# HKUDS/SSLRec

Measured on AMD Instinct MI355X. Metric: propagation_edges_per_sec, higher is better.
Workload: dtype f32

## Files before the change

include/sslrec_hip.h:

```cpp
#ifndef SSLREC_HIP_H
#define SSLREC_HIP_H

#include <stddef.h>
#include <stdint.h>

#ifdef __cplusplus
extern "C" {
#endif

#define SSLREC_ABI_VERSION 7
#define SSLREC_E_BADARG 1001

int sslrec_abi_version(void);

int sslrec_row_bits3(const int64_t *idx0, int64_t off0, const int64_t *idx1, int64_t off1, const int64_t *idx2, int64_t off2,
                     int32_t n, int32_t n_rows, uint32_t *bits, void *stream);

typedef struct sslrec_csr {
    int32_t n_rows, n_cols, nnz;
    int32_t d;
    int32_t n_elem;
    const int32_t *col;
    const float   *val;
    int32_t n_waves;
// ... 118 lines not shown
                             int32_t *w_len_out, void *stream);

typedef struct sslrec_plan sslrec_plan_t;
#define SSLREC_PLAN_AUTO 0
#define SSLREC_PLAN_SWEPT 1
#define SSLREC_PLAN_STREAMED 2
#define SSLREC_PLAN_BUNDLED 3
#define SSLREC_PLAN_NO_XCD_SPLIT 1
typedef struct sslrec_plan_info {
    int32_t n_rows, n_cols; int64_t nnz;
    int32_t kind, d, xcd_split;
    int32_t n_elem, n_blocks, n_slots, n_streams, n_rseg, n_long;
    int64_t xcd_col_pairs;
} sslrec_plan_info_t;
int sslrec_plan_build_coo(const int64_t *rows, const int64_t *cols, const float *vals, int64_t nnz, int32_t n_rows,
                          int32_t n_cols, sslrec_plan_t **out);
int sslrec_plan_build_csr(const int64_t *rowptr, const int32_t *col, const float *val, int32_t n_rows, int32_t n_cols,
                          sslrec_plan_t **out);
int sslrec_plan_set_option(sslrec_plan_t *p, const char *name, int64_t value);
int sslrec_plan_layout(sslrec_plan_t *p, int32_t d, int32_t kind, int32_t flags);
int sslrec_plan_info(const sslrec_plan_t *p, int32_t d, int32_t kind, sslrec_plan_info_t *info);
int sslrec_plan_host_array(const sslrec_plan_t *p, int32_t d, int32_t kind, const char *name, const void **ptr, int64_t *count,
                           int32_t *elem_bytes);
int sslrec_plan_upload(sslrec_plan_t *p, int32_t d, int32_t kind, void *stream);
const sslrec_swept_t *sslrec_plan_swept(const sslrec_plan_t *p, int32_t d);
const sslrec_csr_t *sslrec_plan_csr(const sslrec_plan_t *p, int32_t d);
const sslrec_bundled_t *sslrec_plan_bundled(const sslrec_plan_t *p, int32_t d);
const int32_t *sslrec_plan_edge_map(const sslrec_plan_t *p, int32_t d, int32_t kind);
int sslrec_plan_spmm_f32(const sslrec_plan_t *p, int32_t d, const float *X, float *Y, const sslrec_epilogue_t *epi,
                         void *stream);
void sslrec_plan_free(sslrec_plan_t *p);

int sslrec_debug_swept_trace(int enable, unsigned long long *host_out, int n_waves);

int sslrec_debug_stamp_next_launch(unsigned long long *record);
int sslrec_debug_wall_clock_khz(void);

size_t sslrec_bpr_ws_bytes(int32_t B);
size_t sslrec_bpr_bwd_ws_bytes(int32_t B, int32_t d);
int sslrec_bpr_fwd_f32(const float *Ta, const int64_t *ia, const float *Tp, const int64_t *ip,
                       const float *Tn, const int64_t *in, int32_t B, int32_t d, int32_t variant,
                       float divisor, float *ws, float *loss_out, void *stream);
int sslrec_bpr_fwd_total_f32(const float *Ta, const int64_t *ia, const float *Tp, const int64_t *ip,
                             const float *Tn, const int64_t *in, int32_t B, int32_t d, int32_t variant,
                             float divisor, const float *add_in, float *ws, float *loss_out2, void *stream);
int sslrec_bpr_bwd_f32(const float *Ta, const int64_t *ia, const float *Tp, const int64_t *ip,
                       const float *Tn, const int64_t *in, int32_t B, int32_t d, int32_t variant, float divisor,
                       const float *gscale_dev, float *dTa, float *dTp, float *dTn, void *ws, void *stream);
int sslrec_bpr_bwd_table_init(void *ws, int32_t B, int32_t d, void *stream);
int sslrec_bpr_bwd_kept_f32(const float *Ta, const int64_t *ia, const float *Tp, const int64_t *ip,
                            const float *Tn, const int64_t *in, int32_t B, int32_t d, int32_t variant, float divisor,
                            const float *gscale_dev, float *dTa, float *dTp, float *dTn, void *ws, float *zero_table,
                            size_t zero_elems, void *stream);

#define SSLREC_INFONCE_PREC_DEFAULT 0
#define SSLREC_INFONCE_PREC_X6 1
#define SSLREC_INFONCE_PREC_FP32 2
#define SSLREC_INFONCE_PREC_X36 3
#define SSLREC_INFONCE_PREC_X3 4
#define SSLREC_INFONCE_PREC_X63 5
#define SSLREC_INFONCE_PREC_X6A 6
#define SSLREC_INFONCE_PREC_H3 7
#define SSLREC_INFONCE_FWD_W (1 << 16)
size_t sslrec_infonce_ws_bytes(int32_t B, int32_t M, int32_t d);
int sslrec_infonce_fwd_f32(const float *T1, const int64_t *i1, const float *T2, const int64_t *i2,
                           int32_t B, const float *ALL, int32_t M, int32_t d, float temp,
                           int32_t variant, float *ws, float *loss_out, void *stream);
int sslrec_infonce_bwd_f32(const float *T1, const int64_t *i1, const float *T2, const int64_t *i2,
                           int32_t B, const float *ALL, int32_t M, int32_t d, float temp,
                           int32_t variant, float *ws, const float *gscale_dev,
                           float *dE1, float *dE2, float *dALL, void *stream);

int sslrec_infonce_bwd_scatter_f32(const float *T1, const int64_t *i1, const float *T2, const int64_t *i2,
                                   int32_t B, const float *ALL, int32_t M, int32_t d, float temp,
                                   int32_t variant, float *ws, const float *gscale_dev, float *dE,
                                   float *dT1, float *dT2, float *dALL, void *scatter_ws, void *stream);

int sslrec_infonce_shard_rowsum_f32(const float *T1, const int64_t *i1, const float *T2, const int64_t *i2,
                                    int32_t B, const float *ALL, int32_t M, int32_t d, float temp,
                                    int32_t variant, float *ws, float *z_part, void *stream);
int sslrec_infonce_shard_loss_f32(int32_t B, int32_t M, int32_t d, int32_t variant, float *ws,
                                  const float *z_total, float *loss_out, void *stream);
int sslrec_infonce_shard_bwd_f32(int32_t B, int32_t M, int32_t d, float temp, int32_t variant, float *ws,
                                 const float *gscale_dev, float *w_part, float *dALL, void *stream);
int sslrec_infonce_shard_finish_bwd_f32(int32_t B, int32_t M, int32_t d, float temp, int32_t variant,
                                        float *ws, const float *gscale_dev, const float *w_total,
                                        float *dE1, float *dE2, void *stream);

size_t sslrec_sumsq_ws_bytes(void);
int sslrec_sumsq_fwd_f32(const float *x, size_t n, float weight, float *ws, float *out, void *stream);
int sslrec_sumsq_bwd_f32(const float *x, size_t n, float weight, const float *gscale_dev, float *dx, void *stream);

int sslrec_weighted_sum4_f32(const float *t0, float w0, const float *t1, float w1, const float *t2, float w2, const float *t3, float w3,
                             float *out6, void *stream);
int sslrec_scalar_scale2_f32(const float *x, float a, float b, float *out2, void *stream);
int sslrec_add_tables_f32(const float *a, const float *b, const float *c, float *out, size_t n, void *stream);

int sslrec_adam_tick(float *state, double lr, double beta1, double beta2, void *stream);
int sslrec_adam_apply_f32(float *p, const float *g, float *m, float *v, size_t n, const float *state,
                          double beta1, double beta2, double eps, double weight_decay, void *stream);

size_t sslrec_rankq_ws_bytes(int32_t q, int32_t d);
int sslrec_rankq_reduce_f32(const float *M, int64_t stride_q, int64_t stride_n, const float *X, int32_t N, int32_t d,
                            int32_t q, float *ws, float *out, void *stream);
int sslrec_rankq_expand_f32(const float *M, int64_t stride_q, int64_t stride_n, const float *S, int32_t N, int32_t d,
                            int32_t q, float *Y, void *stream);
// ... 27 lines not shown
```

sslrec_amd/_lib.py:

```python
import ctypes as C
import os
import subprocess

_HERE = os.path.dirname(os.path.abspath(__file__))
CSRC = os.path.join(_HERE, 'csrc')
SO_PATH = os.environ.get('SSLREC_HIP_LIBRARY') or os.path.join(CSRC, 'libsslrec_hip.so')

E_BADARG = 1001
EXPECTED_ABI = 7


class CsrStruct(C.Structure):
    _fields_ = [
        ('n_rows', C.c_int32), ('n_cols', C.c_int32), ('nnz', C.c_int32), ('d', C.c_int32), ('n_elem', C.c_int32),
        ('col', C.c_void_p), ('val', C.c_void_p),
        ('n_waves', C.c_int32),
        ('w_start', C.c_void_p), ('w_len', C.c_void_p), ('r_ptr', C.c_void_p),
        ('n_rseg', C.c_int32),
        ('r_len', C.c_void_p), ('r_dst', C.c_void_p),
        ('n_long', C.c_int32),
        ('long_row', C.c_void_p), ('long_ptr', C.c_void_p),
        ('n_slots', C.c_int32),
    ]

# ... 55 lines not shown
    'sslrec_debug_stamp_next_launch': (C.c_int, [C.c_void_p]),
    'sslrec_debug_wall_clock_khz': (C.c_int, []),
    'sslrec_philox_row_sumsq': (C.c_int, [_P, C.c_uint32, _I, _I, _P, _P]),
    'sslrec_row_sumsq_f32': (C.c_int, [_P, _I, _I, _P, _P]),
    'sslrec_debug_gather_rows': (C.c_int, [_P, C.c_uint32, _I, _I, _I, _P, _P, _P]),
    'sslrec_debug_swept_trace': (C.c_int, [C.c_int, _P, C.c_int]),
    'sslrec_spmm_csr_f32': (C.c_int, [C.POINTER(CsrStruct), _P, _P, _P, _P, _P, _I, _P, C.POINTER(EpilogueStruct), _P, _P]),
    'sslrec_spmm_bundled_f32': (C.c_int, [C.POINTER(BundledStruct), _P, _P, _I, _P, C.POINTER(EpilogueStruct), _P, _P]),
    'sslrec_spmm_swept_f32': (C.c_int, [C.POINTER(SweptStruct), _P, _P, _P, _P, _I, _P, C.POINTER(EpilogueStruct), _P]),
    'sslrec_swept_deferred_sum_ok': (C.c_int, [C.POINTER(SweptStruct)]),
    'sslrec_spmm_swept_views_f32': (C.c_int, [C.POINTER(SweptStruct), _P, _I, C.POINTER(EpilogueViewsStruct), _P]),
    'sslrec_swept_compact': (C.c_int, [C.POINTER(SweptStruct), _P, _P, _F, _P, _P, _P, _P]),
    'sslrec_edge_drop_compact': (C.c_int, [C.POINTER(CsrStruct), _P, _P, _F, _P, _P, _P, _P, _P]),
    'sslrec_full_predict_f32': (C.c_int, [_P, _P, _I, _P, _I, _I, _P, _I, _P, _P]),
    'sslrec_eval_topk_ws_bytes': (C.c_size_t, [_I, _I, _I]),
    'sslrec_eval_topk_f32': (C.c_int, [_P, _P, _I, _P, _I, _I, _P, _P, _I, _P, _P, _P, _P]),
    'sslrec_sample_negs': (C.c_int, [_P, C.c_int64, _P, _P, _I, _P, C.c_uint32, _P, _P]),
    'sslrec_sample_negs_mt19937': (C.c_int, [_P, _P, _P, C.c_int64, _P, _P, _I, _I, _P, _P]),
    'sslrec_philox_advance': (C.c_int, [_P, _P]),
    'sslrec_philox_fill_f32': (C.c_int, [_P, C.c_uint32, _P, C.c_size_t, _P]),
    'sslrec_mt19937_uniform_f32': (C.c_int, [_P, _P, C.c_int64, _P]),
    'sslrec_mt19937_keep_mask': (C.c_int, [_P, C.c_float, _P, C.c_int64, _P]),
    'sslrec_mt19937_jump_poly': (C.c_int, [_P, _P, _P, _P]),
    'sslrec_mt19937_par_ws_bytes': (C.c_size_t, [C.c_int32, C.c_int32]),
    'sslrec_mt19937_uniform_par_f32': (C.c_int, [_P, _P, C.c_int32, C.c_int32, C.c_int64, _P, _P, C.c_int64, _P]),
    'sslrec_mt19937_keep_mask_par': (C.c_int, [_P, _P, C.c_int32, C.c_int32, C.c_int64, _P, C.c_float, _P, C.c_int64, _P]),
    'sslrec_swept_compact_philox': (C.c_int, [C.POINTER(SweptStruct), _P, _F, _P, C.c_uint32, _F, _P, _P, _P, _P]),
    'sslrec_edge_drop_compact_philox': (C.c_int, [C.POINTER(CsrStruct), _P, _F, _P, C.c_uint32, _F, _P, _P, _P, _P, _P]),
    'sslrec_bundled_drop_values': (C.c_int, [C.POINTER(BundledStruct), _P, _P, _F, _P, C.c_uint32, _F, _P, _P]),
    'sslrec_bundled_compact': (C.c_int, [C.POINTER(BundledStruct), _P, _P, _F, _P, _P, _P, _P, _P]),
    'sslrec_bundled_compact_philox': (C.c_int, [C.POINTER(BundledStruct), _P, _F, _P, C.c_uint32, _F, _P, _P, _P, _P, _P]),
    'sslrec_spmm_bundled_view_f32': (C.c_int, [C.POINTER(BundledStruct), _P, _P, _P, _P, _P, _I, _P, C.POINTER(EpilogueStruct), _P, _P]),
    'sslrec_plan_build_coo': (C.c_int, [_P, _P, _P, C.c_int64, _I, _I, C.POINTER(C.c_void_p)]),
    'sslrec_plan_build_csr': (C.c_int, [_P, _P, _P, _I, _I, C.POINTER(C.c_void_p)]),
    'sslrec_plan_set_option': (C.c_int, [_P, C.c_char_p, C.c_int64]),
    'sslrec_plan_layout': (C.c_int, [_P, _I, _I, _I]),
    'sslrec_plan_info': (C.c_int, [_P, _I, _I, C.POINTER(PlanInfoStruct)]),
    'sslrec_plan_host_array': (C.c_int, [_P, _I, _I, C.c_char_p, C.POINTER(C.c_void_p), C.POINTER(C.c_int64), C.POINTER(C.c_int32)]),
    'sslrec_plan_upload': (C.c_int, [_P, _I, _I, _P]),
    'sslrec_plan_swept': (C.c_void_p, [_P, _I]),
    'sslrec_plan_csr': (C.c_void_p, [_P, _I]),
    'sslrec_plan_bundled': (C.c_void_p, [_P, _I]),
    'sslrec_plan_edge_map': (C.c_void_p, [_P, _I, _I]),
    'sslrec_plan_spmm_f32': (C.c_int, [_P, _I, _P, _P, C.POINTER(EpilogueStruct), _P]),
    'sslrec_plan_free': (None, [_P]),
    'sslrec_bpr_ws_bytes': (C.c_size_t, [_I]),
    'sslrec_bpr_fwd_f32': (C.c_int, [_P, _P, _P, _P, _P, _P, _I, _I, _I, _F, _P, _P, _P]),
    'sslrec_bpr_fwd_total_f32': (C.c_int, [_P, _P, _P, _P, _P, _P, _I, _I, _I, _F, _P, _P, _P, _P]),
    'sslrec_bpr_bwd_ws_bytes': (C.c_size_t, [_I, _I]),
    'sslrec_scatter_ws_bytes': (C.c_size_t, [_I]),
    'sslrec_bpr_bwd_f32': (C.c_int, [_P, _P, _P, _P, _P, _P, _I, _I, _I, _F, _P, _P, _P, _P, _P, _P]),
    'sslrec_bpr_bwd_table_init': (C.c_int, [_P, _I, _I, _P]),
    'sslrec_bpr_bwd_kept_f32': (C.c_int, [_P, _P, _P, _P, _P, _P, _I, _I, _I, _F, _P, _P, _P, _P, _P, _P, C.c_size_t, _P]),
    'sslrec_infonce_ws_bytes': (C.c_size_t, [_I, _I, _I]),
    'sslrec_infonce_fwd_f32': (C.c_int, [_P, _P, _P, _P, _I, _P, _I, _I, _F, _I, _P, _P, _P]),
    'sslrec_infonce_bwd_f32': (C.c_int, [_P, _P, _P, _P, _I, _P, _I, _I, _F, _I, _P, _P, _P, _P, _P, _P]),
    'sslrec_infonce_bwd_scatter_f32': (C.c_int, [_P, _P, _P, _P, _I, _P, _I, _I, _F, _I, _P, _P, _P, _P, _P, _P, _P, _P]),
    'sslrec_infonce_shard_rowsum_f32': (C.c_int, [_P, _P, _P, _P, _I, _P, _I, _I, _F, _I, _P, _P, _P]),
    'sslrec_infonce_shard_loss_f32': (C.c_int, [_I, _I, _I, _I, _P, _P, _P, _P]),
    'sslrec_infonce_shard_bwd_f32': (C.c_int, [_I, _I, _I, _F, _I, _P, _P, _P, _P, _P]),
    'sslrec_infonce_shard_finish_bwd_f32': (C.c_int, [_I, _I, _I, _F, _I, _P, _P, _P, _P, _P, _P]),
    'sslrec_adam_tick': (C.c_int, [_P, C.c_double, C.c_double, C.c_double, _P]),
    'sslrec_adam_apply_f32': (C.c_int, [_P, _P, _P, _P, C.c_size_t, _P, C.c_double, C.c_double, C.c_double, C.c_double, _P]),
    'sslrec_rankq_ws_bytes': (C.c_size_t, [_I, _I]),
    'sslrec_rankq_reduce_f32': (C.c_int, [_P, C.c_int64, C.c_int64, _P, _I, _I, _I, _P, _P, _P]),
    'sslrec_rankq_expand_f32': (C.c_int, [_P, C.c_int64, C.c_int64, _P, _I, _I, _I, _P, _P]),
    'sslrec_scatter_add_rows_f32': (C.c_int, [_P, _P, _I, _I, _P, _P, _P]),
    'sslrec_sumsq_ws_bytes': (C.c_size_t, []),
    'sslrec_sumsq_fwd_f32': (C.c_int, [_P, C.c_size_t, _F, _P, _P, _P]),
    'sslrec_sumsq_bwd_f32': (C.c_int, [_P, C.c_size_t, _F, _P, _P, _P]),
    'sslrec_weighted_sum4_f32': (C.c_int, [_P, _F, _P, _F, _P, _F, _P, _F, _P, _P]),
    'sslrec_scalar_scale2_f32': (C.c_int, [_P, _F, _F, _P, _P]),
    'sslrec_add_tables_f32': (C.c_int, [_P, _P, _P, _P, C.c_size_t, _P]),
}

_lib = None


def build(force=False):
    if force and os.path.exists(SO_PATH):
        os.remove(SO_PATH)
    subprocess.run(['make', '-C', CSRC], check=True)
    return SO_PATH


def load():
    global _lib
    if _lib is not None:
        return _lib
    if not os.path.exists(SO_PATH):
        raise RuntimeError(
            'libsslrec_hip.so is not built (%s). Run `python __graft_entry__.py` or `make -C sslrec_amd/csrc`. '
            'sslrec_amd has no CPU / PyTorch fallback for its kernels by design.' % SO_PATH)
    lib = C.CDLL(SO_PATH)
    for name, (res, args) in SIGNATURES.items():
        fn = getattr(lib, name)
        fn.restype = res
        fn.argtypes = args
    got = lib.sslrec_abi_version()
    if got != EXPECTED_ABI:
        raise RuntimeError('%s implements ABI version %d, these bindings expect %d: rebuild the library '
                           '(`make -C sslrec_amd/csrc` or `python __graft_entry__.py`)' % (SO_PATH, got, EXPECTED_ABI))
    _lib = lib
    return lib


# ... 5 lines not shown
```

sslrec_amd/csrc/losses.hip:

```cpp
#include "common.h"
#include "det_scatter.h"
#include <stdlib.h>

typedef float f32x4 __attribute__((ext_vector_type(4)));

#define BPR_BLOCKS 256

__device__ __forceinline__ float bpr_term(float x, int variant) {
    if (variant == 0) {
        return (x > 20.f) ? x : log1pf(expf(x));
    }
    return -logf(1.f / (1.f + expf(x)));
}

__device__ __forceinline__ float bpr_dterm(float x, int variant) {
    if (variant == 0 && x > 20.f) return 1.f;
    return 1.f / (1.f + expf(-x));
}

__device__ __forceinline__ int64_t row_of(const int64_t *idx, int b) { return idx ? idx[b] : (int64_t)b; }

#if defined(__HIP_DEVICE_COMPILE__) && !defined(__gfx950__) && !defined(__gfx942__)
#error "finish_by_last_block relies on gfx942 / gfx950 atomics completing at the coherence point: use release / acquire on this target"
#endif
// ... 39 lines not shown
        int last = 0;
        if (atomicInc(reinterpret_cast<unsigned *>(ws + 32 * (g + 1)), (unsigned)size_g - 1u) == (unsigned)size_g - 1u)
            last = atomicInc(reinterpret_cast<unsigned *>(ws), (unsigned)n_groups - 1u) == (unsigned)n_groups - 1u;
        is_last = last;
    }
    __syncthreads();
    if (!is_last) return;
    float v = 0.f;
    for (int i = threadIdx.x; i < n_blocks; i += 256) v += __hip_atomic_load(part + i, __ATOMIC_RELAXED, __HIP_MEMORY_SCOPE_AGENT);
    s[threadIdx.x] = v;
    __syncthreads();
    for (int o = 128; o > 0; o >>= 1) {
        if ((int)threadIdx.x < o) s[threadIdx.x] += s[threadIdx.x + o];
        __syncthreads();
    }
    if (threadIdx.x == 0) {
        const float r = (mul * s[0]) / div;
        out[0] = r;
        if (add_in) out[1] = r + add_in[0];
    }
}

__global__ __launch_bounds__(256) void bpr_fwd_kernel(const float *Ta, const int64_t *ia, const float *Tp,
                                                      const int64_t *ip, const float *Tn, const int64_t *in,
                                                      int B, int d, int variant, float *ws, float divisor, const float *add_in, float *out,
                                                      int one_launch) {
    __shared__ float wsum[4];
    const int lane = threadIdx.x & 63;
    const int w = wave_in_block();
    float local = 0.f;
    for (int b = blockIdx.x * 4 + w; b < B; b += gridDim.x * 4) {
        const float *a = Ta + row_of(ia, b) * d;
        const float *p = Tp + row_of(ip, b) * d;
        const float *n = Tn + row_of(in, b) * d;
        float dp = 0.f, dn = 0.f;
        for (int k = lane; k < d; k += 64) {
            const float av = a[k];
            dp = fmaf(av, p[k], dp);
            dn = fmaf(av, n[k], dn);
        }
        dp = wave_sum(dp);
        dn = wave_sum(dn);
        local += bpr_term(dn - dp, variant);
    }
    if (lane == 0) wsum[w] = local;
    __syncthreads();
    finish_by_last_block(ws, (wsum[0] + wsum[1]) + (wsum[2] + wsum[3]), gridDim.x, 1.f, divisor, add_in, out, one_launch);
}

__global__ __launch_bounds__(256) void bpr_bwd_stage_kernel(const float *Ta, const int64_t *ia, const float *Tp,
                                                            const int64_t *ip, const float *Tn, const int64_t *in,
                                                            int B, int d, int variant, float divisor, const float *gscale,
                                                            float *dTa, float *dTp, float *dTn, float *G,
                                                            DetTable tab, int atomic_fallback, f32x4 *zero_tab, size_t zero_n4) {
    const int lane = threadIdx.x & 63;
    const int w = wave_in_block();
    for (size_t i = (size_t)blockIdx.x * 256 + threadIdx.x; i < zero_n4; i += (size_t)gridDim.x * 256) zero_tab[i] = f32x4{0.f, 0.f, 0.f, 0.f};
    const float g = gscale[0] / divisor;
    const int gw = blockIdx.x * 4 + w, nw = gridDim.x * 4;
    for (int b = gw; b < B; b += nw) {
        const int64_t ra = row_of(ia, b), rp = row_of(ip, b), rn = row_of(in, b);
        const float *a = Ta + ra * d;
        const float *p = Tp + rp * d;
        const float *n = Tn + rn * d;
        float dp = 0.f, dn = 0.f;
        for (int k = lane; k < d; k += 64) {
            const float av = a[k];
            dp = fmaf(av, p[k], dp);
            dn = fmaf(av, n[k], dn);
        }
        dp = wave_sum(dp);
        dn = wave_sum(dn);
        const float s = g * bpr_dterm(dn - dp, variant);
        for (int k = lane; k < d; k += 64) {
            const float av = a[k], pv = p[k], nv = n[k];
            const float ga = s * (nv - pv), gp = -s * av, gn = s * av;
            if (atomic_fallback) {
                if (ia) atomicAdd(dTa + ra * d + k, ga); else dTa[ra * d + k] = ga;
                if (ip) atomicAdd(dTp + rp * d + k, gp); else dTp[rp * d + k] = gp;
                if (in) atomicAdd(dTn + rn * d + k, gn); else dTn[rn * d + k] = gn;
            } else {
                if (ia) G[(size_t)(3 * b + 0) * d + k] = ga; else dTa[ra * d + k] = ga;
                if (ip) G[(size_t)(3 * b + 1) * d + k] = gp; else dTp[rp * d + k] = gp;
                if (in) G[(size_t)(3 * b + 2) * d + k] = gn; else dTn[rn * d + k] = gn;
            }
        }
        if (!atomic_fallback && lane < 3) {
            const int64_t *idx = lane == 0 ? ia : lane == 1 ? ip : in;
            float *dst = lane == 0 ? dTa + ra * d : lane == 1 ? dTp + rp * d : dTn + rn * d;
            if (idx) det_insert(tab, dst, 3 * b + lane); else tab.slot_of[3 * b + lane] = -1;
        }
    }
}

__global__ __launch_bounds__(256) void scatter_add_rows_kernel(const float *src, const int64_t *idx, int B,
                                                               int d, float *dst) {
    const int lane = threadIdx.x & 63;
    const int w = wave_in_block();
    for (int b = blockIdx.x * 4 + w; b < B; b += gridDim.x * 4) {
        const int64_t r = idx[b];
        for (int k = lane; k < d; k += 64) atomicAdd(dst + r * d + k, src[(size_t)b * d + k]);
    }
}

__global__ __launch_bounds__(256) void scatter_insert_kernel(const int64_t *idx, int B, int d, float *dst, DetTable tab) {
    for (int i = blockIdx.x * 256 + threadIdx.x; i < B; i += gridDim.x * 256) det_insert(tab, dst + idx[i] * d, i);
}

extern "C" size_t sslrec_bpr_ws_bytes(int32_t B) {
    (void)B;
    return (size_t)(FIN_PART0 + BPR_BLOCKS) * sizeof(float);
}

extern "C" size_t sslrec_bpr_bwd_ws_bytes(int32_t B, int32_t d) {
    if (B <= 0 || d <= 0 || 3 * (size_t)B > DET_MAX) return 16;
    return (size_t)3 * B * d * sizeof(float) + det_ws_bytes(3 * B) + 16;
}

extern "C" size_t sslrec_scatter_ws_bytes(int32_t B) {
    if (B <= 0 || B > DET_MAX) return 16;
    return det_ws_bytes(B) + 16;
}

static int bpr_fwd_any(const float *Ta, const int64_t *ia, const float *Tp, const int64_t *ip, const float *Tn, const int64_t *in, int32_t B,
                       int32_t d, int32_t variant, float divisor, const float *add_in, float *ws, float *loss_out, void *stream) {
    if (!Ta || !Tp || !Tn || !ws || !loss_out || B < 0 || d <= 0 || (variant != 0 && variant != 1) || !(divisor != 0.f))
        return SSLREC_E_BADARG;
    const int one = one_launch_reduce() ? 1 : 0;
    hipLaunchKernelGGL(bpr_fwd_kernel, dim3(BPR_BLOCKS), dim3(256), 0, (hipStream_t)stream, Ta, ia, Tp, ip, Tn, in, B, d,
                       variant, ws, divisor, add_in, loss_out, one);
    SSLREC_LAUNCH_CHECK();
    if (!one) {
        hipLaunchKernelGGL(finish_partials_kernel, dim3(1), dim3(256), 0, (hipStream_t)stream, ws, BPR_BLOCKS, 1.f, divisor, add_in, loss_out);
        SSLREC_LAUNCH_CHECK();
    }
    return 0;
}

extern "C" int sslrec_bpr_fwd_f32(const float *Ta, const int64_t *ia, const float *Tp, const int64_t *ip,
                                  const float *Tn, const int64_t *in, int32_t B, int32_t d, int32_t variant,
                                  float divisor, float *ws, float *loss_out, void *stream) {
    return bpr_fwd_any(Ta, ia, Tp, ip, Tn, in, B, d, variant, divisor, nullptr, ws, loss_out, stream);
}

extern "C" int sslrec_bpr_fwd_total_f32(const float *Ta, const int64_t *ia, const float *Tp, const int64_t *ip,
                                        const float *Tn, const int64_t *in, int32_t B, int32_t d, int32_t variant,
                                        float divisor, const float *add_in, float *ws, float *loss_out2, void *stream) {
    if (!add_in) return SSLREC_E_BADARG;
    return bpr_fwd_any(Ta, ia, Tp, ip, Tn, in, B, d, variant, divisor, add_in, ws, loss_out2, stream);
}

static int bpr_bwd_any(const float *Ta, const int64_t *ia, const float *Tp, const int64_t *ip,
                       const float *Tn, const int64_t *in, int32_t B, int32_t d, int32_t variant, float divisor,
                       const float *gscale_dev, float *dTa, float *dTp, float *dTn, void *ws, void *stream, bool kept_clean,
                       float *zero_table = nullptr, size_t zero_elems = 0) {
    if (!Ta || !Tp || !Tn || !gscale_dev || !dTa || !dTp || !dTn || B < 0 || d <= 0 ||
        (variant != 0 && variant != 1) || !(divisor != 0.f))
        return SSLREC_E_BADARG;
    if (B == 0) return 0;
    hipStream_t st = (hipStream_t)stream;
    int blocks = (B + 3) / 4;
    if (blocks > 2048) blocks = 2048;
    const bool indexed = ia || ip || in;
    const bool det = indexed && ws && 3 * (size_t)B <= DET_MAX && d <= 256;
    if (!det) {
        if (zero_table) return SSLREC_E_BADARG;
        hipLaunchKernelGGL(bpr_bwd_stage_kernel, dim3(blocks), dim3(256), 0, st, Ta, ia, Tp, ip, Tn, in, B, d, variant, divisor,
                           gscale_dev, dTa, dTp, dTn, (float *)nullptr, DetTable{}, 1, (f32x4 *)nullptr, (size_t)0);
        SSLREC_LAUNCH_CHECK();
        return 0;
    }
    if (zero_table && (!ia || !ip || !in || (zero_elems & 3) || ((uintptr_t)zero_table & 15))) return SSLREC_E_BADARG;
    float *G = (float *)ws;
    const DetTable tab = det_table(G + (size_t)3 * B * d);
    if (!kept_clean) {
        hipLaunchKernelGGL(det_clear_kernel, dim3(64), dim3(256), 0, st, tab);
        SSLREC_LAUNCH_CHECK();
    }
    hipLaunchKernelGGL(bpr_bwd_stage_kernel, dim3(blocks), dim3(256), 0, st, Ta, ia, Tp, ip, Tn, in, B, d, variant, divisor,
                       gscale_dev, dTa, dTp, dTn, G, tab, 0, reinterpret_cast<f32x4 *>(zero_table), zero_elems / 4);
    SSLREC_LAUNCH_CHECK();
    return det_reduce(tab, 3 * B, G, d, st, kept_clean ? 1 : 0);
}

extern "C" int sslrec_bpr_bwd_f32(const float *Ta, const int64_t *ia, const float *Tp, const int64_t *ip,
                                  const float *Tn, const int64_t *in, int32_t B, int32_t d, int32_t variant, float divisor,
                                  const float *gscale_dev, float *dTa, float *dTp, float *dTn, void *ws, void *stream) {
    return bpr_bwd_any(Ta, ia, Tp, ip, Tn, in, B, d, variant, divisor, gscale_dev, dTa, dTp, dTn, ws, stream, false);
}

extern "C" int sslrec_bpr_bwd_table_init(void *ws, int32_t B, int32_t d, void *stream) {
    if (!ws || B <= 0 || d <= 0 || 3 * (size_t)B > DET_MAX || d > 256) return SSLREC_E_BADARG;
    hipLaunchKernelGGL(det_clear_kernel, dim3(64), dim3(256), 0, (hipStream_t)stream, det_table((float *)ws + (size_t)3 * B * d));
    SSLREC_LAUNCH_CHECK();
    return 0;
}

extern "C" int sslrec_bpr_bwd_kept_f32(const float *Ta, const int64_t *ia, const float *Tp, const int64_t *ip,
                                       const float *Tn, const int64_t *in, int32_t B, int32_t d, int32_t variant, float divisor,
                                       const float *gscale_dev, float *dTa, float *dTp, float *dTn, void *ws, float *zero_table,
                                       size_t zero_elems, void *stream) {
    if (!ws || 3 * (size_t)B > DET_MAX || d > 256) return SSLREC_E_BADARG;
    return bpr_bwd_any(Ta, ia, Tp, ip, Tn, in, B, d, variant, divisor, gscale_dev, dTa, dTp, dTn, ws, stream, true, zero_table, zero_elems);
}

extern "C" int sslrec_scatter_add_rows_f32(const float *src, const int64_t *idx, int32_t B, int32_t d,
                                           float *dst, void *ws, void *stream) {
    if (!src || !idx || !dst || B < 0 || d <= 0) return SSLREC_E_BADARG;
    if (B == 0) return 0;
    hipStream_t st = (hipStream_t)stream;
    if (!ws || B > DET_MAX || d > 256) {
        int blocks = (B + 3) / 4;
        if (blocks > 2048) blocks = 2048;
        hipLaunchKernelGGL(scatter_add_rows_kernel, dim3(blocks), dim3(256), 0, st, src, idx, B, d, dst);
        SSLREC_LAUNCH_CHECK();
        return 0;
    }
    const DetTable tab = det_table(ws);
    hipLaunchKernelGGL(det_clear_kernel, dim3(64), dim3(256), 0, st, tab);
    SSLREC_LAUNCH_CHECK();
    hipLaunchKernelGGL(scatter_insert_kernel, dim3((B + 255) / 256), dim3(256), 0, st, idx, B, d, dst, tab);
    SSLREC_LAUNCH_CHECK();
    return det_reduce(tab, B, src, d, st);
}

#define SUMSQ_BLOCKS 1024

__global__ __launch_bounds__(256) void sumsq_kernel(const float *x, size_t n, float *ws, float weight, float *out, int one_launch) {
    __shared__ float wsum[4];
    const int lane = threadIdx.x & 63;
    float acc = 0.f;
    const size_t n4 = n / 4;
    const f32x4 *x4 = reinterpret_cast<const f32x4 *>(x);
    for (size_t i = (size_t)blockIdx.x * 256 + threadIdx.x; i < n4; i += (size_t)gridDim.x * 256) {
        const f32x4 v = x4[i];
        acc = fmaf(v[0], v[0], acc);
        acc = fmaf(v[1], v[1], acc);
        acc = fmaf(v[2], v[2], acc);
        acc = fmaf(v[3], v[3], acc);
    }
    if (blockIdx.x == 0 && threadIdx.x < (n & 3)) {
        const float v = x[n4 * 4 + threadIdx.x];
        acc = fmaf(v, v, acc);
    }
    acc = wave_sum(acc);
    if (lane == 0) wsum[threadIdx.x >> 6] = acc;
    __syncthreads();
    finish_by_last_block(ws, (wsum[0] + wsum[1]) + (wsum[2] + wsum[3]), gridDim.x, weight, 1.f, nullptr, out, one_launch);
}

__global__ __launch_bounds__(256) void scale2_kernel(const float *x, size_t n, const float *g, float weight, float *out) {
    const float s = 2.f * (g[0] * weight);
    const size_t n4 = n / 4;
    const f32x4 *x4 = reinterpret_cast<const f32x4 *>(x);
    f32x4 *o4 = reinterpret_cast<f32x4 *>(out);
    for (size_t i = (size_t)blockIdx.x * 256 + threadIdx.x; i < n4; i += (size_t)gridDim.x * 256) {
// ... 376 lines not shown
```

sslrec_amd/ops.py:

```python
import ctypes as C

import os

import torch

from . import _lib
from .graph import BundledLayout, DroppedView, PropGraph, RevaluedView, graph_of

PROFILE = None
PROFILE_EVERY = 1
_profile_tick = 0


def _profile_this_launch():
    global _profile_tick
    if PROFILE is None:
        return False
    _profile_tick += 1
    return PROFILE_EVERY <= 1 or _profile_tick % PROFILE_EVERY == 0


PROFILE_INFONCE = None

STAMPS = None


class StampLog:
    def __init__(self, device, capacity=512):
        self.buf = torch.zeros((capacity, 4), dtype=torch.int64, device=device)
        self.buf[:, 0] = -1
        self.meta = []
        self.khz = int(_lib.load().sslrec_debug_wall_clock_khz())

    def attach_next(self, *meta):
        if len(self.meta) >= self.buf.shape[0]:
            raise RuntimeError('StampLog is full (%d launches)' % self.buf.shape[0])
        rc = _lib.load().sslrec_debug_stamp_next_launch(self.buf[len(self.meta)].data_ptr())
        _lib.check(rc, 'sslrec_debug_stamp_next_launch')
        self.meta.append(meta)

    def reset_counts(self):
        torch.cuda.synchronize(self.buf.device)
        self.buf[:, 1:] = 0
        self.buf[:, 0] = -1
        torch.cuda.synchronize(self.buf.device)

    def read(self):
        host = self.buf.cpu().numpy()
        out = []
        for i, meta in enumerate(self.meta):
            n = int(host[i, 3])
            if n > 0:
                out.append((meta, float(host[i, 1]) / n / self.khz, n))
        return out

# ... 50 lines not shown
    cur = torch.cuda.current_stream(dev)
    ent = _TICKET_WS.get(key)
    if ent is None or ent[0].numel() * 4 < n_bytes:
        ent = _TICKET_WS[key] = [torch.zeros(max(n_bytes // 4, 1), dtype=torch.float32, device=dev), cur]
    elif ent[1] != cur:
        if not torch.cuda.is_current_stream_capturing():
            cur.wait_stream(ent[1])
        ent[1] = cur
    return ent[0]


import collections
import threading

_KEPT_WS = collections.OrderedDict()
_KEPT_WS_MAX = 8
_KEPT_WS_LOCK = threading.Lock()
SSLREC_KEPT_SCATTER = os.environ.get('SSLREC_KEPT_SCATTER', '1') != '0'


def _bpr_bwd_ws(device, B, d):
    lib = _lib.load()
    n = lib.sslrec_bpr_bwd_ws_bytes(B, d) // 4 + 1
    if not SSLREC_KEPT_SCATTER or 3 * B > 16384 or d > 256 or B <= 0:
        return torch.empty(n, dtype=torch.float32, device=device), False
    dev = torch.device(device)
    key = (dev.index if dev.index is not None else torch.cuda.current_device(), int(B), int(d))
    cur = torch.cuda.current_stream(dev)
    with _KEPT_WS_LOCK:
        ent = _KEPT_WS.get(key)
        if ent is None:
            ws = torch.empty(n, dtype=torch.float32, device=dev)
            _lib.check(lib.sslrec_bpr_bwd_table_init(ws.data_ptr(), int(B), int(d), _stream()), 'sslrec_bpr_bwd_table_init')
            ent = _KEPT_WS[key] = [ws, cur]
            while len(_KEPT_WS) > _KEPT_WS_MAX and not torch.cuda.is_current_stream_capturing():
                _k, old_ent = _KEPT_WS.popitem(last=False)
                if old_ent[1] is not None:
                    old_ent[0].record_stream(old_ent[1])
        else:
            _KEPT_WS.move_to_end(key)
            if ent[1] != cur:
                if not torch.cuda.is_current_stream_capturing():
                    cur.wait_stream(ent[1])
                ent[1] = cur
    return ent[0], True


def _check_kept(rc, what, device, B, d):
    if rc != 0:
        dev = torch.device(device)
        with _KEPT_WS_LOCK:
            _KEPT_WS.pop((dev.index if dev.index is not None else torch.cuda.current_device(), int(B), int(d)), None)
    _lib.check(rc, what)


def _need_gpu(*tensors):
    for t in tensors:
        if t is not None and not t.is_cuda:
            raise RuntimeError('sslrec_amd kernels run on a HIP device only (got a %s tensor); there is no CPU '
                               'fallback by design' % t.device)


def _f32c(t):
    if t.dtype != torch.float32:
        raise TypeError('fp32 tensors expected, got %s' % t.dtype)
    return t if t.is_contiguous() else t.contiguous()


def _idx(t):
    if t is None:
        return None
    if t.dtype != torch.int64:
        t = t.long()
    return t if t.is_contiguous() else t.contiguous()


def _ptr(t):
    return 0 if t is None else t.data_ptr()


def spmm_raw(adj, x, which='fwd', y=None, noise=None, eps=0.0, acc_in=None, acc_out=None, want_y=True, chained=False,
             noise_sumsq=None, noise_geom=None, axpy=None, x_row_bits=None, sum_in=None, row_scale=None, scale_flags=0):
    view = adj if isinstance(adj, (DroppedView, RevaluedView)) else None
    graph = adj.graph if view is not None else adj
    plan = getattr(graph, which)
    _need_gpu(x)
    x = _f32c(x)
    n, d = x.shape
    if n != plan.n_cols:
        raise ValueError('operand has %d rows, matrix has %d columns' % (n, plan.n_cols))
    if d not in SPMM_DIMS and d not in SPMM_NARROW_DIMS:
        raise ValueError('embedding size %d not supported by the raw HIP SpMM launcher (supported: %s and %s); the ops.spmm / '
                         'ops.propagate_sum wrappers zero-pad other sizes' % (d, SPMM_NARROW_DIMS, SPMM_DIMS))
    if want_y and y is None:
        y = torch.empty((plan.n_rows, d), dtype=torch.float32, device=x.device)
    epi = None
    keep_alive = []
    if noise is not None or acc_out is not None or x_row_bits is not None or scale_flags:
        epi = _lib.EpilogueStruct()
        if scale_flags:
            if row_scale is None or row_scale.numel() != plan.n_rows or row_scale.dtype != torch.float32 or not row_scale.is_contiguous():
                raise ValueError('row_scale: contiguous fp32 [%d] expected' % plan.n_rows)
            epi.row_scale, epi.scale_flags = row_scale.data_ptr(), int(scale_flags)
        if x_row_bits is not None:
            if x_row_bits.n_rows != n:
                raise ValueError('row bitmap of %d rows for an operand of %d rows' % (x_row_bits.n_rows, n))
# ... 462 lines not shown
    _lib.check(rc, 'sslrec_bpr_bwd_f32')
    return out, da, dp, dn


def bpr_loss(anc, pos, neg, variant=0, divisor=1.0):
    return _BprFn.apply(anc, pos, neg, None, None, None, int(variant), False, float(divisor))


class _BprStackedFn(torch.autograd.Function):

    @staticmethod
    def forward(ctx, table, n_user, ancs, poss, negs, variant, divisor, add):
        _need_gpu(table)
        table = _f32c(table)
        ia, ip, in_ = _idx(ancs), _idx(poss), _idx(negs)
        B, d = int(ia.numel()), table.shape[1]
        lib = _lib.load()
        ws = _ticket_ws(table.device, lib.sslrec_bpr_ws_bytes(B), 'bpr')
        p = table.data_ptr()
        pi = p + int(n_user) * d * 4
        ctx.save_for_backward(table, ia, ip, in_)
        ctx.meta = (B, d, variant, int(n_user), float(divisor))
        ctx.two = add is not None
        ctx.set_materialize_grads(False)
        if add is None:
            out = torch.empty(1, dtype=torch.float32, device=table.device)
            rc = lib.sslrec_bpr_fwd_f32(p, ia.data_ptr(), pi, ip.data_ptr(), pi, in_.data_ptr(), B, d, variant, float(divisor),
                                        ws.data_ptr(), out.data_ptr(), _stream())
            _lib.check(rc, 'sslrec_bpr_fwd_f32')
            return out.reshape(())
        _need_gpu(add)
        addc = add.detach().reshape(1).to(torch.float32).contiguous()
        out = torch.empty(2, dtype=torch.float32, device=table.device)
        rc = lib.sslrec_bpr_fwd_total_f32(p, ia.data_ptr(), pi, ip.data_ptr(), pi, in_.data_ptr(), B, d, variant, float(divisor),
                                          addc.data_ptr(), ws.data_ptr(), out.data_ptr(), _stream())
        _lib.check(rc, 'sslrec_bpr_fwd_total_f32')
        return out[1].reshape(()), out[0].reshape(())

    @staticmethod
    def backward(ctx, *grads):
        table, ia, ip, in_ = ctx.saved_tensors
        B, d, variant, n_user, divisor = ctx.meta
        if ctx.two:
            g_total, g_bpr = grads
            g_add = g_total
            g = g_total if g_bpr is None else (g_bpr if g_total is None else g_total + g_bpr)
        else:
            g, g_add = grads[0], None
        if g is None:
            return None, None, None, None, None, None, None, g_add
        g = g.reshape(1).to(torch.float32).contiguous()
        lib = _lib.load()
        ws, kept = _bpr_bwd_ws(table.device, B, d)
        fused_zero = kept and B > 0 and table.numel() % 4 == 0
        grad = torch.empty_like(table) if fused_zero else torch.zeros_like(table)
        p, q = table.data_ptr(), grad.data_ptr()
        pi, qi = p + n_user * d * 4, q + n_user * d * 4
        args = (p, ia.data_ptr(), pi, ip.data_ptr(), pi, in_.data_ptr(), B, d, variant, divisor, g.data_ptr(), q, qi, qi, ws.data_ptr())
        if kept:
            rc = lib.sslrec_bpr_bwd_kept_f32(*args, q if fused_zero else None, grad.numel() if fused_zero else 0, _stream())
        else:
            rc = lib.sslrec_bpr_bwd_f32(*args, _stream())
        _check_kept(rc, 'sslrec_bpr_bwd_f32', table.device, B, d)
        if SPARSE_GRAD:
            _tag_row_bits(grad, RowBits.from_indices(table.shape[0], ia, 0, ip, n_user, in_, n_user))
        return grad, None, None, None, None, None, None, g_add


def bpr_loss_stacked(table, n_user, ancs, poss, negs, variant=0, divisor=1.0, add=None):
    return _BprStackedFn.apply(table, int(n_user), ancs, poss, negs, int(variant), float(divisor), add)


def bpr_loss_gathered(user_table, item_table, ancs, poss, negs, variant=0, divisor=1.0):
    return _BprFn.apply(user_table, item_table, item_table, ancs, poss, negs, int(variant), True, float(divisor))


def _infonce_event():
    if PROFILE_INFONCE is None:
        return None
    ev = torch.cuda.Event(enable_timing=True)
    ev.record()
    return ev


def _infonce_record(ev0, kind, B, M, d, variant):
    if ev0 is not None and PROFILE_INFONCE is not None:
        ev1 = torch.cuda.Event(enable_timing=True)
        ev1.record()
        PROFILE_INFONCE.append((ev0, ev1, kind, B, M, d, variant))


def infonce_issued_flops(kind, B, M, d, variant):
    code = (variant >> 8) & 0xFF
    v1 = (variant & 0xFF) != 0
    if code == 0:
        v1_default = 'x6' if (os.environ.get('SSLREC_INFONCE_V1_DEFAULT') or 'h3')[0] == 'x' else 'h3'
        code = INFONCE_PRECISIONS.get(os.environ.get('SSLREC_INFONCE_PRECISION') or (v1_default if v1 else 'h3'), 1)
    if v1 and code not in (2, 7):
        code = 1
    fwd_w = bool(variant & INFONCE_FWD_W_BIT) and not (code == 2 and d == 128)
    sc, wa, da = {1: (6, 6, 6), 2: (1, 1, 1), 3: (3, 6, 6), 4: (3, 3, 3), 5: (6, 3, 3), 6: (6, 6, 3), 7: (3, 3, 3)}[code]
    unit = 2.0 * B * M * d
    pre = 1 if (v1 and code == 7 and (kind == 'fwd')) else 0
    if kind == 'fwd':
        f = sc + (wa if fwd_w else 0) + pre
    else:
        f = sc + da + (0 if fwd_w else sc + wa)
    return f * unit, ('fp32' if code == 2 else ('fp16' if code == 7 else 'bf16'))


class _InfoNceFn(torch.autograd.Function):
    @staticmethod
# ... 530 lines not shown
```

Measured before the change: 56.30 billion.

## Reuse persistent BPR gradient buffer and clear only previously touched rows

Instead of zeroing the whole embedding-table gradient on every BPR backward, a cached gradient tensor is kept per (device, shape, B). The kernel zeroes only the rows written in the previous call, which it recorded as offsets, and then records the rows it writes now. This avoids a full-table memset per step, at the cost of returning an aliased persistent tensor whose exclusivity is checked with refcount, use_count and version heuristics. If that check misses a live reference, results can be silently wrong.

```diff
diff --git a/include/sslrec_hip.h b/include/sslrec_hip.h
--- a/include/sslrec_hip.h
+++ b/include/sslrec_hip.h
@@ -194,6 +194,10 @@
                             const float *Tn, const int64_t *in, int32_t B, int32_t d, int32_t variant, float divisor,
                             const float *gscale_dev, float *dTa, float *dTp, float *dTn, void *ws, float *zero_table,
                             size_t zero_elems, void *stream);
+int sslrec_bpr_bwd_kept_rows_f32(const float *Ta, const int64_t *ia, const float *Tp, const int64_t *ip,
+                                 const float *Tn, const int64_t *in, int32_t B, int32_t d, int32_t variant, float divisor,
+                                 const float *gscale_dev, float *dTa, float *dTp, float *dTn, void *ws, float *table,
+                                 size_t table_elems, int64_t *rows, void *stream);
 
 #define SSLREC_INFONCE_PREC_DEFAULT 0
 #define SSLREC_INFONCE_PREC_X6 1
diff --git a/sslrec_amd/_lib.py b/sslrec_amd/_lib.py
--- a/sslrec_amd/_lib.py
+++ b/sslrec_amd/_lib.py
@@ -131,6 +131,7 @@
     'sslrec_bpr_bwd_f32': (C.c_int, [_P, _P, _P, _P, _P, _P, _I, _I, _I, _F, _P, _P, _P, _P, _P, _P]),
     'sslrec_bpr_bwd_table_init': (C.c_int, [_P, _I, _I, _P]),
     'sslrec_bpr_bwd_kept_f32': (C.c_int, [_P, _P, _P, _P, _P, _P, _I, _I, _I, _F, _P, _P, _P, _P, _P, _P, C.c_size_t, _P]),
+    'sslrec_bpr_bwd_kept_rows_f32': (C.c_int, [_P, _P, _P, _P, _P, _P, _I, _I, _I, _F, _P, _P, _P, _P, _P, _P, C.c_size_t, _P, _P]),
     'sslrec_infonce_ws_bytes': (C.c_size_t, [_I, _I, _I]),
     'sslrec_infonce_fwd_f32': (C.c_int, [_P, _P, _P, _P, _I, _P, _I, _I, _F, _I, _P, _P, _P]),
     'sslrec_infonce_bwd_f32': (C.c_int, [_P, _P, _P, _P, _I, _P, _I, _I, _F, _I, _P, _P, _P, _P, _P, _P]),
diff --git a/sslrec_amd/csrc/losses.hip b/sslrec_amd/csrc/losses.hip
--- a/sslrec_amd/csrc/losses.hip
+++ b/sslrec_amd/csrc/losses.hip
@@ -115,13 +115,22 @@
                                                             const int64_t *ip, const float *Tn, const int64_t *in,
                                                             int B, int d, int variant, float divisor, const float *gscale,
                                                             float *dTa, float *dTp, float *dTn, float *G,
-                                                            DetTable tab, int atomic_fallback, f32x4 *zero_tab, size_t zero_n4) {
+                                                            DetTable tab, int atomic_fallback, f32x4 *zero_tab, size_t zero_n4,
+                                                            float *clear_base, int64_t *clear_rows) {
     const int lane = threadIdx.x & 63;
     const int w = wave_in_block();
     for (size_t i = (size_t)blockIdx.x * 256 + threadIdx.x; i < zero_n4; i += (size_t)gridDim.x * 256) zero_tab[i] = f32x4{0.f, 0.f, 0.f, 0.f};
     const float g = gscale[0] / divisor;
     const int gw = blockIdx.x * 4 + w, nw = gridDim.x * 4;
     for (int b = gw; b < B; b += nw) {
+        if (clear_rows) {
+            const int64_t o0 = clear_rows[3 * (size_t)b], o1 = clear_rows[3 * (size_t)b + 1], o2 = clear_rows[3 * (size_t)b + 2];
+            for (int k = lane; k < d; k += 64) {
+                if (o0 >= 0) clear_base[o0 + k] = 0.f;
+                if (o1 >= 0) clear_base[o1 + k] = 0.f;
+                if (o2 >= 0) clear_base[o2 + k] = 0.f;
+            }
+        }
         const int64_t ra = row_of(ia, b), rp = row_of(ip, b), rn = row_of(in, b);
         const float *a = Ta + ra * d;
         const float *p = Tp + rp * d;
@@ -152,6 +161,7 @@
             const int64_t *idx = lane == 0 ? ia : lane == 1 ? ip : in;
             float *dst = lane == 0 ? dTa + ra * d : lane == 1 ? dTp + rp * d : dTn + rn * d;
             if (idx) det_insert(tab, dst, 3 * b + lane); else tab.slot_of[3 * b + lane] = -1;
+            if (clear_rows) clear_rows[3 * (size_t)b + lane] = (int64_t)(dst - clear_base);
         }
     }
 }
@@ -216,7 +226,7 @@
 static int bpr_bwd_any(const float *Ta, const int64_t *ia, const float *Tp, const int64_t *ip,
                        const float *Tn, const int64_t *in, int32_t B, int32_t d, int32_t variant, float divisor,
                        const float *gscale_dev, float *dTa, float *dTp, float *dTn, void *ws, void *stream, bool kept_clean,
-                       float *zero_table = nullptr, size_t zero_elems = 0) {
+                       float *zero_table = nullptr, size_t zero_elems = 0, float *clear_base = nullptr, int64_t *clear_rows = nullptr) {
     if (!Ta || !Tp || !Tn || !gscale_dev || !dTa || !dTp || !dTn || B < 0 || d <= 0 ||
         (variant != 0 && variant != 1) || !(divisor != 0.f))
         return SSLREC_E_BADARG;
@@ -227,9 +237,10 @@
     const bool indexed = ia || ip || in;
     const bool det = indexed && ws && 3 * (size_t)B <= DET_MAX && d <= 256;
     if (!det) {
-        if (zero_table) return SSLREC_E_BADARG;
+        if (zero_table || clear_rows) return SSLREC_E_BADARG;
         hipLaunchKernelGGL(bpr_bwd_stage_kernel, dim3(blocks), dim3(256), 0, st, Ta, ia, Tp, ip, Tn, in, B, d, variant, divisor,
-                           gscale_dev, dTa, dTp, dTn, (float *)nullptr, DetTable{}, 1, (f32x4 *)nullptr, (size_t)0);
+                           gscale_dev, dTa, dTp, dTn, (float *)nullptr, DetTable{}, 1, (f32x4 *)nullptr, (size_t)0, (float *)nullptr,
+                           (int64_t *)nullptr);
         SSLREC_LAUNCH_CHECK();
         return 0;
     }
@@ -241,7 +252,7 @@
         SSLREC_LAUNCH_CHECK();
     }
     hipLaunchKernelGGL(bpr_bwd_stage_kernel, dim3(blocks), dim3(256), 0, st, Ta, ia, Tp, ip, Tn, in, B, d, variant, divisor,
-                       gscale_dev, dTa, dTp, dTn, G, tab, 0, reinterpret_cast<f32x4 *>(zero_table), zero_elems / 4);
+                       gscale_dev, dTa, dTp, dTn, G, tab, 0, reinterpret_cast<f32x4 *>(zero_table), zero_elems / 4, clear_base, clear_rows);
     SSLREC_LAUNCH_CHECK();
     return det_reduce(tab, 3 * B, G, d, st, kept_clean ? 1 : 0);
 }
@@ -265,6 +276,16 @@
                                        size_t zero_elems, void *stream) {
     if (!ws || 3 * (size_t)B > DET_MAX || d > 256) return SSLREC_E_BADARG;
     return bpr_bwd_any(Ta, ia, Tp, ip, Tn, in, B, d, variant, divisor, gscale_dev, dTa, dTp, dTn, ws, stream, true, zero_table, zero_elems);
+}
+
+extern "C" int sslrec_bpr_bwd_kept_rows_f32(const float *Ta, const int64_t *ia, const float *Tp, const int64_t *ip,
+                                            const float *Tn, const int64_t *in, int32_t B, int32_t d, int32_t variant, float divisor,
+                                            const float *gscale_dev, float *dTa, float *dTp, float *dTn, void *ws, float *table,
+                                            size_t table_elems, int64_t *rows, void *stream) {
+    if (!ws || !table || !rows || !ia || !ip || !in || 3 * (size_t)B > DET_MAX || d > 256) return SSLREC_E_BADARG;
+    const float *lo = table, *hi = table + table_elems;
+    if (!dTa || !dTp || !dTn || dTa < lo || dTp < lo || dTn < lo || dTa >= hi || dTp >= hi || dTn >= hi) return SSLREC_E_BADARG;
+    return bpr_bwd_any(Ta, ia, Tp, ip, Tn, in, B, d, variant, divisor, gscale_dev, dTa, dTp, dTn, ws, stream, true, nullptr, 0, table, rows);
 }
 
 extern "C" int sslrec_scatter_add_rows_f32(const float *src, const int64_t *idx, int32_t B, int32_t d,
diff --git a/sslrec_amd/ops.py b/sslrec_amd/ops.py
--- a/sslrec_amd/ops.py
+++ b/sslrec_amd/ops.py
@@ -1,6 +1,7 @@
 import ctypes as C
 
 import os
+import sys
 
 import torch
 
@@ -157,6 +158,51 @@
         with _KEPT_WS_LOCK:
             _KEPT_WS.pop((dev.index if dev.index is not None else torch.cuda.current_device(), int(B), int(d)), None)
     _lib.check(rc, what)
+
+
+_KEPT_GRAD = collections.OrderedDict()
+_KEPT_GRAD_MAX = 2
+SSLREC_KEPT_GRAD = os.environ.get('SSLREC_KEPT_GRAD', '1') != '0'
+
+
+def _exclusive(ent):
+    return sys.getrefcount(ent[0]) <= 2 and ent[0]._use_count() == 1 and ent[0]._version == ent[3]
+
+
+def _kept_grad(table, B):
+    if not (SSLREC_KEPT_GRAD and SSLREC_KEPT_SCATTER) or table.grad_fn is None or B <= 0 or 3 * B > 16384 or table.shape[1] > 256:
+        return None
+    dev = table.device
+    key = (dev.index if dev.index is not None else torch.cuda.current_device(), int(table.shape[0]), int(table.shape[1]), int(B))
+    cur = torch.cuda.current_stream(dev)
+    with _KEPT_WS_LOCK:
+        ent = _KEPT_GRAD.get(key)
+        if ent is not None and not _exclusive(ent):
+            del _KEPT_GRAD[key]
+            ent[0].record_stream(ent[2])
+            ent = None
+        if ent is None:
+            grad = torch.zeros(table.shape, dtype=torch.float32, device=dev)
+            rows = torch.full((3 * B,), -1, dtype=torch.int64, device=dev)
+            ent = _KEPT_GRAD[key] = [grad, rows, cur, grad._version]
+            while len(_KEPT_GRAD) > _KEPT_GRAD_MAX and not torch.cuda.is_current_stream_capturing():
+                _k, old = _KEPT_GRAD.popitem(last=False)
+                old[0].record_stream(old[2])
+                old[1].record_stream(old[2])
+        else:
+            _KEPT_GRAD.move_to_end(key)
+            if ent[2] != cur:
+                if not torch.cuda.is_current_stream_capturing():
+                    cur.wait_stream(ent[2])
+                ent[2] = cur
+        return ent[0], ent[1]
+
+
+def _drop_kept_grad(table, B):
+    dev = table.device
+    with _KEPT_WS_LOCK:
+        _KEPT_GRAD.pop((dev.index if dev.index is not None else torch.cuda.current_device(), int(table.shape[0]), int(table.shape[1]), int(B)),
+                       None)
 
 
 def _need_gpu(*tensors):
@@ -725,12 +771,17 @@
         g = g.reshape(1).to(torch.float32).contiguous()
         lib = _lib.load()
         ws, kept = _bpr_bwd_ws(table.device, B, d)
-        fused_zero = kept and B > 0 and table.numel() % 4 == 0
-        grad = torch.empty_like(table) if fused_zero else torch.zeros_like(table)
+        kg = _kept_grad(table, B) if kept else None
+        fused_zero = kg is None and kept and B > 0 and table.numel() % 4 == 0
+        grad = kg[0] if kg is not None else torch.empty_like(table) if fused_zero else torch.zeros_like(table)
         p, q = table.data_ptr(), grad.data_ptr()
         pi, qi = p + n_user * d * 4, q + n_user * d * 4
         args = (p, ia.data_ptr(), pi, ip.data_ptr(), pi, in_.data_ptr(), B, d, variant, divisor, g.data_ptr(), q, qi, qi, ws.data_ptr())
-        if kept:
+        if kg is not None:
+            rc = lib.sslrec_bpr_bwd_kept_rows_f32(*args, q, grad.numel(), kg[1].data_ptr(), _stream())
+            if rc != 0:
+                _drop_kept_grad(table, B)
+        elif kept:
             rc = lib.sslrec_bpr_bwd_kept_f32(*args, q if fused_zero else None, grad.numel() if fused_zero else 0, _stream())
         else:
             rc = lib.sslrec_bpr_bwd_f32(*args, _stream())
```

After: 56.66 billion, median of 6. About the same (+0.6%).
